# ramanathanlab/distllm

Measured on NVIDIA H100. Metric: embedded chunks/sec @512-tok, higher is better.
Workload: dtype bf16

## Files before the change

distllm_b200/_native.py:

```python

from __future__ import annotations

import ctypes as C
from pathlib import Path

import torch

LIB_PATH = Path(__file__).resolve().parent / 'libb2e.so'
LIB_PATHS = {'f16': LIB_PATH, 'bf16': LIB_PATH.with_name('libb2e_bf16.so')}
STORAGE_TORCH_DTYPE = {'f16': torch.float16, 'bf16': torch.bfloat16}
_STORAGE_BY_ARCH = {'bert': 'bf16', 'esm': 'bf16', 'modernbert': 'bf16', 'mistral': 'f16', 'qwen3': 'f16'}


def storage_for_arch(arch: str) -> str:
    import os

    forced = os.environ.get('B2E_STORAGE')
    if forced:
        if forced not in LIB_PATHS:
            raise NativeError(f'B2E_STORAGE={forced!r}: expected one of {sorted(LIB_PATHS)}')
        return forced
    return _STORAGE_BY_ARCH[arch]


# ... 17 lines not shown
    'b2e_num_weights',
    'b2e_check_model',
    'b2e_encoder_create',
    'b2e_encoder_create_nf4',
    'b2e_encoder_destroy',
    'b2e_workspace_bytes',
    'b2e_encode',
    'b2e_encode_pooled',
    'b2e_embed_host',
    'b2e_pool_mean',
    'b2e_pool_last_token',
    'b2e_l2_normalize',
    'b2e_adjacent_cosine_dist',
    'b2e_gemm_h16',
    'b2e_gemm_nf4',
    'b2e_attention_d64',
    'b2e_attention_d32',
    'b2e_attention_d64_window',
    'b2e_attention_causal_d128',
    'b2e_qk_norm_rope',
    'b2e_topk_ip',
    'b2e_topk_ip_tc',
    'b2e_max_row_norm',
    'b2e_pack_ubinary',
    'b2e_search_ubinary',
    'b2e_layernorm',
)
DEBUG_EXPORTS = (
    'b2e_debug_set_att3_clock',
    'b2e_debug_set_clock_buffer',
    'b2e_debug_set_layers',
    'b2e_debug_set_att3_variant',
    'b2e_debug_set_packing',
    'b2e_debug_topk_tc_fell_back',
)


class NativeError(RuntimeError):
    """Raised when libb2e.so is missing or a native call fails."""


class ModelDesc(C.Structure):

    _fields_ = [
        ('arch', C.c_int32),
        ('num_layers', C.c_int32),
        ('hidden', C.c_int32),
        ('heads', C.c_int32),
        ('kv_heads', C.c_int32),
        ('head_dim', C.c_int32),
        ('intermediate', C.c_int32),
        ('vocab', C.c_int32),
        ('max_pos', C.c_int32),
        ('type_vocab', C.c_int32),
        ('eps', C.c_float),
        ('rope_theta', C.c_float),
        ('sliding_window', C.c_int32),
        ('reserved', C.c_int32),
        ('rope_theta_local', C.c_float),
        ('global_every', C.c_int32),
    ]


_libs: dict[str, C.CDLL] = {}


# ... 385 lines not shown
```

distllm_b200/csrc/b2e_api.cu:

```cuda
#include "../../include/b2e.h"
#include "../../include/b2e_debug.h"

#include <cuda.h>
#include <cuda_runtime.h>

#include <cstdarg>
#include <cstdio>
#include <cstdlib>
#include <cstring>
#include <string>
#include <utility>
#include <vector>

#include "attention.cuh"
#include "binsearch.cuh"
#include "common.cuh"
#include "gemm.cuh"
#include "mistral_ops.cuh"
#include "pack.cuh"
#include "rowops.cuh"
#include "topk.cuh"
#include "topk_tc.cuh"

using namespace b2e;
// ... 127 lines not shown
  }
  static DeviceInfo cache[64];
  if (dev < 64 && cache[dev].ok) {
    *info = cache[dev];
    return B2E_OK;
  }
  int rc = device_info(dev, info);
  if (rc == B2E_OK && dev < 64) cache[dev] = *info;
  return rc;
}

template <typename Kern>
int ensure_smem_attr(Kern kern, int bytes) {
  static std::vector<std::pair<const void*, int>> done;
  int dev = 0;
  CUDA_TRY(cudaGetDevice(&dev));
  const void* key = reinterpret_cast<const void*>(kern);
  for (const auto& d : done)
    if (d.first == key && d.second == dev) return B2E_OK;
  CUDA_TRY(cudaFuncSetAttribute(kern, cudaFuncAttributeMaxDynamicSharedMemorySize, bytes));
  done.emplace_back(key, dev);
  return B2E_OK;
}

int check_gemm_shape(int M, int N, int K) {
  if (M <= 0 || N <= 0 || K <= 0) return fail(B2E_ERR_INVALID, "gemm: empty shape %dx%dx%d", M, N, K);
  if (N % 128 != 0) return fail(B2E_ERR_INVALID, "gemm: N=%d must be a multiple of 128", N);
  if (K % 64 != 0) return fail(B2E_ERR_INVALID, "gemm: K=%d must be a multiple of 64", K);
  return B2E_OK;
}

bool g_gemm_profiling = false;

struct GemmW {
  CUtensorMap tm;
  const float* absmax = nullptr;
};

int make_gemm_w(GemmW* w, const void* base, const float* absmax, uint64_t rows, uint64_t cols) {
  w->absmax = absmax;
  return absmax ? make_tmap_codes(&w->tm, base, rows, cols / 2) : make_tmap_h16(&w->tm, base, rows, cols, GEMM_BN);
}

template <int EPI>
int launch_gemm_epi(const CUtensorMap& ta, const GemmW& wb, void* out, const float* bias,
                    const h16* resid, int M, int N, int K, cudaStream_t st, const int* m_dev) {
  auto kern = gemm_h16_wgmma_kernel<EPI>;
  int smem = GEMM_SMEM_BYTES;
  if (wb.absmax) {
    kern = gemm_h16_wgmma_kernel<EPI, false, true>;
    smem = GemmPlan<true>::SMEM_BYTES;
  } else if constexpr (EPI == EPI_BIAS) {
    if (g_gemm_profiling) kern = gemm_h16_wgmma_kernel<EPI, true>;
  }
  int rc = ensure_smem_attr(kern, smem);
  if (rc) return rc;
  DeviceInfo dev;
  if ((rc = current_device_info(&dev))) return rc;
  const long long tiles = (long long)(N / GEMM_BN) * ((M + GEMM_BM - 1) / GEMM_BM);
  if (tiles > 0x7fffffffLL) return fail(B2E_ERR_INVALID, "gemm: %lld output tiles exceed one grid", tiles);
  CUtensorMap tm_out;
  if ((rc = make_tmap_h16(&tm_out, out, M, epi_is_glu(EPI) ? N / 2 : N, GEMM_BM))) return rc;
  const unsigned grid = (unsigned)(tiles < dev.sms ? tiles : dev.sms);
  kern<<<grid, GEMM_THREADS, smem, st>>>(ta, wb.tm, tm_out, static_cast<h16*>(out), bias, resid, M, N, K, m_dev,
                                         wb.absmax);
  CUDA_TRY(cudaGetLastError());
  return B2E_OK;
}

int launch_gemm(const CUtensorMap& ta, const GemmW& tb, void* out, const float* bias,
                const void* resid, int M, int N, int K, int epi, cudaStream_t st, const int* m_dev = nullptr) {
  const h16* r = static_cast<const h16*>(resid);
  switch (epi) {
    case B2E_EPI_BIAS: return launch_gemm_epi<EPI_BIAS>(ta, tb, out, bias, r, M, N, K, st, m_dev);
    case B2E_EPI_BIAS_GELU: return launch_gemm_epi<EPI_BIAS_GELU>(ta, tb, out, bias, r, M, N, K, st, m_dev);
    case B2E_EPI_BIAS_RESID: return launch_gemm_epi<EPI_BIAS_RESID>(ta, tb, out, bias, r, M, N, K, st, m_dev);
    case B2E_EPI_SWIGLU: return launch_gemm_epi<EPI_SWIGLU>(ta, tb, out, bias, r, M, N, K, st, m_dev);
    case B2E_EPI_GEGLU: return launch_gemm_epi<EPI_GEGLU>(ta, tb, out, bias, r, M, N, K, st, m_dev);
  }
  return fail(B2E_ERR_INVALID, "unknown epilogue %d", epi);
}

struct AttnScratch {
  float* bias = nullptr;
  int* kv_chunks = nullptr;
  int* plain_chunks = nullptr;
  size_t cap_bias = 0, cap_b = 0;
  uint64_t gen = 0;
  int device = -1;
  int ensure(int B, int S_pad) {
    int dev = 0;
    CUDA_TRY(cudaGetDevice(&dev));
// ... 599 lines not shown
      return rc;
    if ((rc = launch_gemm(tm_ffn, e->tm_w2[l], e->tmp, nullptr, nullptr, M, H, I, B2E_EPI_BIAS, st, lay.t_real)))
      return rc;
  }
  CUDA_TRY(cudaGetLastError());
  return B2E_OK;
}

}

extern "C" {

int b2e_version(void) { return B2E_ABI_VERSION; }
int b2e_storage_dtype(void) { return kStorageDtype; }

int b2e_debug_set_att3_clock(void* device_buffer) {
  long long* p = static_cast<long long*>(device_buffer);
  CUDA_TRY(cudaMemcpyToSymbol(g_att_clock, &p, sizeof(p)));
  return B2E_OK;
}

int b2e_debug_set_att3_variant(int variant) {
  g_att3_variant = variant;
  return B2E_OK;
}

int b2e_debug_set_clock_buffer(void* device_buffer) {
  long long* p = static_cast<long long*>(device_buffer);
  g_gemm_profiling = p != nullptr;
  CUDA_TRY(cudaMemcpyToSymbol(g_gemm_clock, &p, sizeof(p)));
  return B2E_OK;
}

int b2e_debug_set_packing(int on) {
  g_packing = on ? 1 : 0;
  return B2E_OK;
}

int b2e_debug_set_layers(B2EEncoder* e, int n) {
  if (!e) return fail(B2E_ERR_INVALID, "null encoder handle");
  if (n == 0) n = e->full_layers;
  if (n < 1 || n > e->full_layers)
    return fail(B2E_ERR_INVALID, "layer count %d outside [1, %d]", n, e->full_layers);
  if (n != e->desc.num_layers) e->drop_graphs();
  e->desc.num_layers = n;
  return B2E_OK;
}
const char* b2e_last_error(void) { return g_err.c_str(); }

int b2e_num_weights(const B2EModelDesc* desc) {
  if (!desc) return -1;
  if (desc->arch == B2E_ARCH_BERT) return 5 + 12 * desc->num_layers;
  if (desc->arch == B2E_ARCH_ESM2) return 3 + 12 * desc->num_layers;
  if (is_decoder(desc->arch)) return 2 + decoder_layer_slots(desc->arch) * desc->num_layers;
  if (desc->arch == B2E_ARCH_MODERNBERT) return 5 + 8 * desc->num_layers;
  return -1;
}

int b2e_check_model(const B2EModelDesc* desc) {
  if (!desc) return fail(B2E_ERR_INVALID, "null model description");
  if (desc->num_layers <= 0 || desc->hidden <= 0 || desc->heads <= 0 || desc->intermediate <= 0)
    return fail(B2E_ERR_INVALID, "model description has a non-positive size");
  int rc;
  if (is_decoder(desc->arch)) {
    const char* fam = desc->arch == B2E_ARCH_QWEN3 ? "Qwen3" : "Mistral";
    if (desc->head_dim != 128 || desc->kv_heads <= 0 || desc->heads % desc->kv_heads != 0)
// ... 34 lines not shown
                "{1,2,3,4,5,8,10,16}, 384 and 640 (MiniLM / BGE-small / E5-small: 384 = 12 x 32); of the ESM-2 family "
                "that is esm2_t30_150M (H=640), esm2_t33_650M (H=1280) and esm2_t36_3B (H=2560)",
                desc->heads, desc->head_dim, desc->hidden);
  if ((rc = check_h(desc->hidden))) return rc;
  if ((rc = check_gemm_shape(128, 3 * desc->hidden, desc->hidden))) return rc;
  if ((rc = check_gemm_shape(128, desc->intermediate, desc->hidden))) return rc;
  return check_gemm_shape(128, desc->hidden, desc->intermediate);
}

namespace {
int create_mistral(const B2EModelDesc* desc, const void* const* weights, int n_weights, const float* const* absmax,
                   int device, B2EEncoder** out) {
  const int L = desc->num_layers, H = desc->hidden, I = desc->intermediate;
  const int QC = (desc->heads + 2 * desc->kv_heads) * 128, CC = desc->heads * 128;
  int rc;
  if ((rc = b2e_check_model(desc))) return rc;
  if (n_weights != b2e_num_weights(desc))
    return fail(B2E_ERR_INVALID, "expected %d weight pointers, got %d", b2e_num_weights(desc), n_weights);
  for (int i = 0; i < n_weights; ++i)
    if (!weights[i]) return fail(B2E_ERR_INVALID, "weight pointer %d is null", i);
  DeviceInfo info;
  if ((rc = device_info(device, &info))) return rc;
  DeviceGuard guard;
  CUDA_TRY(cudaSetDevice(device));
  B2EEncoder* e = new B2EEncoder();
  e->desc = *desc;
  e->full_layers = desc->num_layers;
  e->w.assign(weights, weights + n_weights);
  e->device = device;
  e->sms = info.sms;
  e->tm_wqkv.resize(L); e->tm_wo.resize(L); e->tm_w1.resize(L); e->tm_w2.resize(L);
  for (int l = 0; l < L; ++l) {
    const float* const* s = absmax ? absmax + 4 * l : nullptr;
    if ((rc = make_gemm_w(&e->tm_wqkv[l], e->Mi(l, 1), s ? s[0] : nullptr, QC, H)) ||
        (rc = make_gemm_w(&e->tm_wo[l], e->Mi(l, 2), s ? s[1] : nullptr, H, CC)) ||
        (rc = make_gemm_w(&e->tm_w1[l], e->Mi(l, 4), s ? s[2] : nullptr, 2 * I, H)) ||
        (rc = make_gemm_w(&e->tm_w2[l], e->Mi(l, 5), s ? s[3] : nullptr, H, I))) {
      delete e;
      return rc;
    }
  }
  const size_t n = (size_t)desc->max_pos * 64;
  if (cudaMalloc(&e->rope_cos, n * sizeof(float)) != cudaSuccess ||
      cudaMalloc(&e->rope_sin, n * sizeof(float)) != cudaSuccess) {
    b2e_encoder_destroy(e);
    return fail(B2E_ERR_CUDA, "cudaMalloc of the rotary tables failed");
  }
  rope_table_theta_kernel<<<(unsigned)((n + 255) / 256), 256>>>(e->rope_cos, e->rope_sin, desc->max_pos,
                                                                64, desc->rope_theta);
  if (cudaDeviceSynchronize() != cudaSuccess) {
    b2e_encoder_destroy(e);
    return fail(B2E_ERR_CUDA, "rotary table kernel failed: %s", cudaGetErrorString(cudaGetLastError()));
  }
  *out = e;
  return B2E_OK;
}
}

namespace {
int create_encoder(const B2EModelDesc* desc, const void* const* weights, int n_weights, const float* const* absmax,
                   int device, B2EEncoder** out) {
  if (!desc || !weights || !out) return fail(B2E_ERR_INVALID, "null argument");
  *out = nullptr;
  if (is_decoder(desc->arch)) return create_mistral(desc, weights, n_weights, absmax, device, out);
  int rc;
  if ((rc = b2e_check_model(desc))) return rc;
  if (n_weights != b2e_num_weights(desc))
    return fail(B2E_ERR_INVALID, "expected %d weight pointers, got %d", b2e_num_weights(desc),
                n_weights);
  for (int i = 0; i < n_weights; ++i)
    if (!weights[i]) return fail(B2E_ERR_INVALID, "weight pointer %d is null", i);
  DeviceInfo info;
  if ((rc = device_info(device, &info))) return rc;
  DeviceGuard guard;
  CUDA_TRY(cudaSetDevice(device));

  B2EEncoder* e = new B2EEncoder();
  e->desc = *desc;
  e->full_layers = desc->num_layers;
  e->w.assign(weights, weights + n_weights);
  e->device = device;
  e->sms = info.sms;
  const int L = desc->num_layers, H = desc->hidden, I = desc->intermediate;
  e->tm_wqkv.resize(L); e->tm_wo.resize(L); e->tm_w1.resize(L); e->tm_w2.resize(L);
  const bool esm = desc->arch == B2E_ARCH_ESM2;
  const bool mbert = desc->arch == B2E_ARCH_MODERNBERT;
  const int n1 = mbert ? 2 * I : I;
  for (int l = 0; l < L; ++l) {
    const void* wqkv = mbert ? e->Mb(l, 2) : esm ? e->E(l, 2) : e->L(l, 0);
    const void* wo = mbert ? e->Mb(l, 3) : esm ? e->E(l, 4) : e->L(l, 2);
    const void* w1 = mbert ? e->Mb(l, 6) : esm ? e->E(l, 8) : e->L(l, 6);
    const void* w2 = mbert ? e->Mb(l, 7) : esm ? e->E(l, 10) : e->L(l, 8);
    const float* const* s = absmax ? absmax + 4 * l : nullptr;
    if ((rc = make_gemm_w(&e->tm_wqkv[l], wqkv, s ? s[0] : nullptr, 3 * H, H)) ||
        (rc = make_gemm_w(&e->tm_wo[l], wo, s ? s[1] : nullptr, H, H)) ||
        (rc = make_gemm_w(&e->tm_w1[l], w1, s ? s[2] : nullptr, n1, H)) ||
        (rc = make_gemm_w(&e->tm_w2[l], w2, s ? s[3] : nullptr, H, I))) {
      delete e;
      return rc;
    }
  }
  if (mbert) {
    const size_t n = (size_t)desc->max_pos * 32;
    if (cudaMalloc(&e->rope_cos, n * sizeof(float)) != cudaSuccess ||
        cudaMalloc(&e->rope_sin, n * sizeof(float)) != cudaSuccess ||
        cudaMalloc(&e->rope_cos2, n * sizeof(float)) != cudaSuccess ||
        cudaMalloc(&e->rope_sin2, n * sizeof(float)) != cudaSuccess) {
      b2e_encoder_destroy(e);
      return fail(B2E_ERR_CUDA, "cudaMalloc of the rotary tables failed");
    }
    rope_table_theta_kernel<<<(unsigned)((n + 255) / 256), 256>>>(e->rope_cos, e->rope_sin, desc->max_pos, 32,
                                                                  desc->rope_theta);
    rope_table_theta_kernel<<<(unsigned)((n + 255) / 256), 256>>>(e->rope_cos2, e->rope_sin2, desc->max_pos, 32,
                                                                  desc->rope_theta_local);
    if (cudaDeviceSynchronize() != cudaSuccess) {
      b2e_encoder_destroy(e);
      return fail(B2E_ERR_CUDA, "rotary table kernel failed: %s", cudaGetErrorString(cudaGetLastError()));
    }
  }
  if (esm) {
    const size_t n = (size_t)desc->max_pos * 32;
    if (cudaMalloc(&e->rope_cos, n * sizeof(float)) != cudaSuccess ||
        cudaMalloc(&e->rope_sin, n * sizeof(float)) != cudaSuccess) {
      b2e_encoder_destroy(e);
      return fail(B2E_ERR_CUDA, "cudaMalloc of the rotary tables failed");
    }
    if (desc->head_dim == 32)
      rope_table_theta_kernel<<<(unsigned)((n / 2 + 255) / 256), 256>>>(e->rope_cos, e->rope_sin, desc->max_pos, 16,
                                                                        10000.0f);
    else
// ... 371 lines not shown
  switch (dtype) {
    case B2E_DTYPE_F32:
      adjacent_cosine_kernel<float><<<blocks, 256, 0, st>>>((const float*)emb, doc_id, out,
                                                            (int)n_rows, H);
      break;
    case B2E_DTYPE_BF16:
      adjacent_cosine_kernel<bf16><<<blocks, 256, 0, st>>>((const bf16*)emb, doc_id, out,
                                                           (int)n_rows, H);
      break;
    case B2E_DTYPE_F16:
      adjacent_cosine_kernel<__half><<<blocks, 256, 0, st>>>((const __half*)emb, doc_id, out,
                                                             (int)n_rows, H);
      break;
    default:
      return fail(B2E_ERR_INVALID, "adjacent_cosine_dist: dtype %d", dtype);
  }
  CUDA_TRY(cudaGetLastError());
  return B2E_OK;
}

int b2e_gemm_h16(const void* A, const void* W, const float* bias, const void* resid, void* out,
                  int M, int N, int K, int epi, void* stream) {
  if (!A || !W || !out) return fail(B2E_ERR_INVALID, "null tensor pointer");
  if (epi == B2E_EPI_BIAS_RESID && !resid) return fail(B2E_ERR_INVALID, "resid epilogue needs resid");
  int rc;
  if ((rc = check_gemm_shape(M, N, K))) return rc;
  if ((epi == B2E_EPI_SWIGLU || epi == B2E_EPI_GEGLU) && N % 256 != 0)
    return fail(B2E_ERR_INVALID, "gemm: the gated epilogues need N %% 256 == 0 (got %d)", N);
  DeviceInfo info;
  if ((rc = current_device_info(&info))) return rc;
  CUtensorMap ta;
  GemmW tb;
  if ((rc = make_tmap_h16(&ta, A, M, K, 128))) return rc;
  if ((rc = make_gemm_w(&tb, W, nullptr, N, K))) return rc;
  return launch_gemm(ta, tb, out, bias, resid, M, N, K, epi, (cudaStream_t)stream);
}

int b2e_gemm_nf4(const void* A, const void* codes, const float* absmax, const float* bias, const void* resid,
                 void* out, int M, int N, int K, int epi, void* stream) {
  if (!A || !codes || !absmax || !out) return fail(B2E_ERR_INVALID, "null tensor pointer");
  if (reinterpret_cast<uintptr_t>(absmax) % 16 != 0) return fail(B2E_ERR_INVALID, "absmax not 16-byte aligned");
  if (epi == B2E_EPI_BIAS_RESID && !resid) return fail(B2E_ERR_INVALID, "resid epilogue needs resid");
  int rc;
  if ((rc = check_gemm_shape(M, N, K))) return rc;
  if ((epi == B2E_EPI_SWIGLU || epi == B2E_EPI_GEGLU) && N % 256 != 0)
    return fail(B2E_ERR_INVALID, "gemm: the gated epilogues need N %% 256 == 0 (got %d)", N);
  DeviceInfo info;
  if ((rc = current_device_info(&info))) return rc;
  CUtensorMap ta;
  GemmW tb;
  if ((rc = make_tmap_h16(&ta, A, M, K, 128))) return rc;
  if ((rc = make_gemm_w(&tb, codes, absmax, N, K))) return rc;
  return launch_gemm(ta, tb, out, bias, resid, M, N, K, epi, (cudaStream_t)stream);
}

int b2e_attention_d64(const void* qkv, const int64_t* mask, void* ctx, int B, int S, int heads,
                      float* dbg, void* stream) {
  if (!qkv || !mask || !ctx) return fail(B2E_ERR_INVALID, "null tensor pointer");
  if (B <= 0 || S <= 0 || heads <= 0) return fail(B2E_ERR_INVALID, "empty attention problem");
  if (dbg) return fail(B2E_ERR_UNSUPPORTED, "the score dump of the first attention kernel is gone: pass NULL");
  int rc;
  DeviceInfo info;
  if ((rc = current_device_info(&info))) return rc;
  cudaStream_t st = (cudaStream_t)stream;
  CUtensorMap tkv;
  if ((rc = make_tmap_h16(&tkv, qkv, (uint64_t)B * S, (uint64_t)3 * heads * 64, AT_KC))) return rc;
  if ((rc = attention_prepare(g_attn_scratch, mask, B, S, st))) return rc;
  return launch_attention(tkv, g_attn_scratch, ctx, B, S, heads, st);
}

int b2e_attention_d32(const void* qkv, const int64_t* mask, void* ctx, int B, int S, int heads, void* stream) {
  if (!qkv || !mask || !ctx) return fail(B2E_ERR_INVALID, "null tensor pointer");
  if (B <= 0 || S <= 0 || heads <= 0) return fail(B2E_ERR_INVALID, "empty attention problem");
  int rc;
  DeviceInfo info;
  if ((rc = current_device_info(&info))) return rc;
  cudaStream_t st = (cudaStream_t)stream;
  CUtensorMap tkv;
  if ((rc = make_tmap_h16(&tkv, qkv, (uint64_t)B * S, (uint64_t)3 * heads * 32, AT_KC, 32))) return rc;
  if ((rc = attention_prepare(g_attn_scratch, mask, B, S, st))) return rc;
  return launch_attention_bidir(tkv, g_attn_scratch, ctx, B, S, heads, 32, st);
}

int b2e_attention_d64_window(const void* qkv, const int64_t* mask, void* ctx, int B, int S, int heads,
                             int window, void* stream) {
// ... 385 lines not shown
```

distllm_b200/csrc/common.cuh:

```cuda
#pragma once

#include <cuda.h>
#include <cuda_bf16.h>
#include <cuda_fp16.h>
#include <cuda_runtime.h>
#include <stdint.h>

namespace b2e {

using bf16 = __nv_bfloat16;
#ifdef B2E_STORAGE_BF16
using h16 = __nv_bfloat16;
#else
using h16 = __half;
#endif

__device__ __forceinline__ uint32_t smem_u32(const void* p) {
  return static_cast<uint32_t>(__cvta_generic_to_shared(p));
}

__device__ __forceinline__ uint32_t lane_id() { return threadIdx.x & 31u; }

__device__ __forceinline__ bool elect_one() {
  uint32_t pred = 0;
// ... 186 lines not shown
        "+f"(d[24]), "+f"(d[25]), "+f"(d[26]), "+f"(d[27]), "+f"(d[28]), "+f"(d[29]), "+f"(d[30]), "+f"(d[31])
      : "r"(a[0]), "r"(a[1]), "r"(a[2]), "r"(a[3]), "l"(b));
}

__device__ __forceinline__ void wgmma_64x32_rs_tb(float (&d)[16], const uint32_t (&a)[4], uint64_t b) {
  asm volatile(
      "{\n.reg .pred p;\nsetp.eq.u32 p, 1, 1;\n"
      "wgmma.mma_async.sync.aligned.m64n32k16.f32." B2E_WGMMA_AB " "
      "{%0,%1,%2,%3,%4,%5,%6,%7,%8,%9,%10,%11,%12,%13,%14,%15}, {%16,%17,%18,%19}, %20, p, 1, 1, 1;\n}\n"
      : "+f"(d[0]), "+f"(d[1]), "+f"(d[2]), "+f"(d[3]), "+f"(d[4]), "+f"(d[5]), "+f"(d[6]), "+f"(d[7]),
        "+f"(d[8]), "+f"(d[9]), "+f"(d[10]), "+f"(d[11]), "+f"(d[12]), "+f"(d[13]), "+f"(d[14]), "+f"(d[15])
      : "r"(a[0]), "r"(a[1]), "r"(a[2]), "r"(a[3]), "l"(b));
}

__device__ __forceinline__ void wgmma_64x128_ss(float (&d)[64], uint64_t a, uint64_t b, int accumulate) {
  asm volatile(
      "{\n.reg .pred p;\nsetp.ne.b32 p, %66, 0;\n"
      "wgmma.mma_async.sync.aligned.m64n128k16.f32." B2E_WGMMA_AB " "
      "{%0,%1,%2,%3,%4,%5,%6,%7,%8,%9,%10,%11,%12,%13,%14,%15,"
      "%16,%17,%18,%19,%20,%21,%22,%23,%24,%25,%26,%27,%28,%29,%30,%31,"
      "%32,%33,%34,%35,%36,%37,%38,%39,%40,%41,%42,%43,%44,%45,%46,%47,"
      "%48,%49,%50,%51,%52,%53,%54,%55,%56,%57,%58,%59,%60,%61,%62,%63}, %64, %65, p, 1, 1, 0, 0;\n}\n"
      : "+f"(d[0]), "+f"(d[1]), "+f"(d[2]), "+f"(d[3]), "+f"(d[4]), "+f"(d[5]), "+f"(d[6]), "+f"(d[7]),
        "+f"(d[8]), "+f"(d[9]), "+f"(d[10]), "+f"(d[11]), "+f"(d[12]), "+f"(d[13]), "+f"(d[14]), "+f"(d[15]),
        "+f"(d[16]), "+f"(d[17]), "+f"(d[18]), "+f"(d[19]), "+f"(d[20]), "+f"(d[21]), "+f"(d[22]), "+f"(d[23]),
        "+f"(d[24]), "+f"(d[25]), "+f"(d[26]), "+f"(d[27]), "+f"(d[28]), "+f"(d[29]), "+f"(d[30]), "+f"(d[31]),
        "+f"(d[32]), "+f"(d[33]), "+f"(d[34]), "+f"(d[35]), "+f"(d[36]), "+f"(d[37]), "+f"(d[38]), "+f"(d[39]),
        "+f"(d[40]), "+f"(d[41]), "+f"(d[42]), "+f"(d[43]), "+f"(d[44]), "+f"(d[45]), "+f"(d[46]), "+f"(d[47]),
        "+f"(d[48]), "+f"(d[49]), "+f"(d[50]), "+f"(d[51]), "+f"(d[52]), "+f"(d[53]), "+f"(d[54]), "+f"(d[55]),
        "+f"(d[56]), "+f"(d[57]), "+f"(d[58]), "+f"(d[59]), "+f"(d[60]), "+f"(d[61]), "+f"(d[62]), "+f"(d[63])
      : "l"(a), "l"(b), "r"(accumulate));
}

__device__ __forceinline__ void wgmma_64x16_tf32(float (&d)[8], uint64_t a, uint64_t b, int accumulate) {
  asm volatile(
      "{\n.reg .pred p;\nsetp.ne.b32 p, %10, 0;\n"
      "wgmma.mma_async.sync.aligned.m64n16k8.f32.tf32.tf32 {%0,%1,%2,%3,%4,%5,%6,%7}, %8, %9, p, 1, 1;\n}\n"
      : "+f"(d[0]), "+f"(d[1]), "+f"(d[2]), "+f"(d[3]), "+f"(d[4]), "+f"(d[5]), "+f"(d[6]), "+f"(d[7])
      : "l"(a), "l"(b), "r"(accumulate));
}


__device__ __forceinline__ uint32_t pack_h16x2(float lo, float hi) {
  uint32_t r;
#ifdef B2E_STORAGE_BF16
  asm("cvt.rn.bf16x2.f32 %0, %1, %2;" : "=r"(r) : "f"(hi), "f"(lo));
#else
  asm("cvt.rn.satfinite.f16x2.f32 %0, %1, %2;" : "=r"(r) : "f"(hi), "f"(lo));
#endif
  return r;
}
__device__ __forceinline__ float2 unpack_h16x2(uint32_t u) {
#ifdef B2E_STORAGE_BF16
  __nv_bfloat162 v = *reinterpret_cast<__nv_bfloat162*>(&u);
  return __bfloat1622float2(v);
#else
  __half2 v = *reinterpret_cast<__half2*>(&u);
  return __half22float2(v);
#endif
}
__device__ __forceinline__ float2 unpack_bf16x2(uint32_t u) {
  __nv_bfloat162 v = *reinterpret_cast<__nv_bfloat162*>(&u);
  return __bfloat1622float2(v);
}
__device__ __forceinline__ h16 to_h16(float x) {
#ifdef B2E_STORAGE_BF16
// ... 32 lines not shown
```

distllm_b200/csrc/gemm.cuh:

```cuda
#pragma once

#include "common.cuh"

namespace b2e {

enum GemmEpi : int { EPI_BIAS = 0, EPI_BIAS_GELU = 1, EPI_BIAS_RESID = 2, EPI_SWIGLU = 3, EPI_GEGLU = 4 };
__host__ __device__ constexpr bool epi_is_glu(int epi) { return epi == EPI_SWIGLU || epi == EPI_GEGLU; }

constexpr int GEMM_BM = 128;
constexpr int GEMM_BN = 128;
constexpr int GEMM_BK = 64;
constexpr int GEMM_STAGES = 5;
constexpr int GEMM_THREADS = 384;
constexpr int GEMM_PRODUCER_REGS = 40, GEMM_CONSUMER_REGS = 232;
constexpr int GEMM_A_BYTES = GEMM_BM * GEMM_BK * 2;
constexpr int GEMM_STAGE_BYTES = GEMM_A_BYTES + GEMM_BN * GEMM_BK * 2;
constexpr int GEMM_OUT_BOX = GEMM_BM * 64 * 2;
constexpr int GEMM_OUT_OFFSET = GEMM_STAGES * GEMM_STAGE_BYTES;
constexpr int GEMM_BAR_OFFSET = GEMM_OUT_OFFSET + 2 * 2 * GEMM_OUT_BOX;
constexpr int GEMM_SMEM_BYTES = GEMM_BAR_OFFSET + 16 * GEMM_STAGES + 1024;
static_assert(GEMM_SMEM_BYTES <= 232448, "shared memory of one SM");
constexpr int GEMM_BAR_TURN = 1, GEMM_BAR_STAGE = 3, GEMM_BAR_NF4 = 5;

constexpr int GEMM_NF4_RAW = 4;
constexpr int GEMM_NF4_CODE_BYTES = GEMM_BN * GEMM_BK / 2;
constexpr int GEMM_NF4_RAW_BYTES = GEMM_NF4_CODE_BYTES + GEMM_BN * 4;

template <bool NF4>
struct GemmPlan {
  static constexpr int STAGES = NF4 ? 4 : GEMM_STAGES;
  static constexpr int OUT_OFFSET = STAGES * GEMM_STAGE_BYTES;
  static constexpr int RAW_OFFSET = OUT_OFFSET + 2 * 2 * GEMM_OUT_BOX;
  static constexpr int BAR_OFFSET = RAW_OFFSET + (NF4 ? GEMM_NF4_RAW * GEMM_NF4_RAW_BYTES : 0);
  static constexpr int TABLE_OFFSET = BAR_OFFSET + 16 * STAGES + (NF4 ? 8 * GEMM_NF4_RAW : 0);
  static constexpr int SMEM_BYTES = TABLE_OFFSET + (NF4 ? 16 * 4 : 0) + 1024;
  static constexpr int PRODUCER_REGS = NF4 ? 56 : GEMM_PRODUCER_REGS;
  static constexpr int CONSUMER_REGS = NF4 ? 224 : GEMM_CONSUMER_REGS;
  static_assert(128 * PRODUCER_REGS + 256 * CONSUMER_REGS <= GEMM_THREADS * 168, "registers the CTA holds");
  static_assert(SMEM_BYTES <= 232448, "shared memory of one SM");
};
static_assert(GemmPlan<false>::SMEM_BYTES == GEMM_SMEM_BYTES && GemmPlan<false>::BAR_OFFSET == GEMM_BAR_OFFSET,
              "the 16-bit plan");

__constant__ uint32_t kNf4CodeBits[16] = {
    0xbf800000u, 0xbf3239b1u, 0xbf066b30u, 0xbeca32a0u, 0xbe91a24du, 0xbe3d353fu, 0xbdba7871u, 0x00000000u,
    0x3da2faffu, 0x3e24cae3u, 0x3e7c04ddu, 0x3ead033au, 0x3ee1a4b8u, 0x3f1007abu, 0x3f3913b3u, 0x3f800000u,
};

__device__ __forceinline__ float gelu_erf_fast(float x) {
  const float xc = fminf(fmaxf(x, -5.65685f), 5.65685f);
  const float v = xc * xc;
  float q = fmaf(v, -1.35688221e-05f, -1.95764464e-04f);
  q = fmaf(v, q, 3.65498251e-02f);
  q = fmaf(v, q, 7.97818838e-01f);
  float t;
  asm("tanh.approx.f32 %0, %1;" : "=f"(t) : "f"(xc * q));
  const float h = 0.5f * x;
  return fmaf(h, t, h);
}

__device__ __forceinline__ float gelu_erf(float x) {
  const float ax = fabsf(x);
  float t;
  asm("rcp.approx.ftz.f32 %0, %1;" : "=f"(t) : "f"(fmaf(0.3275911f * 0.70710678f, ax, 1.0f)));
  float p = fmaf(t, 1.061405429f, -1.453152027f);
  p = fmaf(t, p, 1.421413741f);
  p = fmaf(t, p, -0.284496736f);
  p = fmaf(t, p, 0.254829592f);
  p *= t;
  const float e = fast_exp2(ax * ax * (-0.5f * 1.4426950408889634f));
  return fmaxf(x, 0.0f) - 0.5f * ax * p * e;
}

__device__ __forceinline__ float silu(float x) {
  float r;
  asm("rcp.approx.ftz.f32 %0, %1;" : "=f"(r) : "f"(1.0f + fast_exp2(-1.4426950408889634f * x)));
  return x * r;
}


__device__ long long* g_gemm_clock = nullptr;

struct GemmTiles {
  int first, stride, count, n_tiles;
};
__device__ __forceinline__ GemmTiles gemm_tiles(int M, int N) {
  const int n_tiles = N / GEMM_BN;
  const int tiles = n_tiles * ((M + GEMM_BM - 1) / GEMM_BM);
  const int first = static_cast<int>(blockIdx.x), stride = static_cast<int>(gridDim.x);
  return {first, stride, first < tiles ? (tiles - 1 - first) / stride + 1 : 0, n_tiles};
}

__device__ __forceinline__ float ld_shared_const_f32(uint32_t addr) {
  float v;
  asm("ld.shared.f32 %0, [%1];" : "=f"(v) : "r"(addr));
  return v;
}
__device__ __forceinline__ float ld_shared_f32(uint32_t addr) {
  float v;
  asm volatile("ld.shared.f32 %0, [%1];" : "=f"(v) : "r"(addr) : "memory");
  return v;
}
__device__ __forceinline__ uint4 ld_shared_v4(uint32_t addr) {
  uint4 v;
  asm volatile("ld.shared.v4.u32 {%0, %1, %2, %3}, [%4];" : "=r"(v.x), "=r"(v.y), "=r"(v.z), "=r"(v.w) : "r"(addr)
               : "memory");
  return v;
}
__device__ __forceinline__ void st_shared_v4(uint32_t addr, uint32_t a, uint32_t b, uint32_t c, uint32_t d) {
  asm volatile("st.shared.v4.b32 [%0], {%1, %2, %3, %4};" ::"r"(addr), "r"(a), "r"(b), "r"(c), "r"(d) : "memory");
}

__device__ __forceinline__ void gemm_nf4_producer(const CUtensorMap* tm_a, const CUtensorMap* tm_codes,
                                                  const float* __restrict__ absmax, const GemmTiles& tl, int N,
                                                  int kblocks, uint32_t sb, uint32_t full_bar, uint32_t empty_bar) {
  using P = GemmPlan<true>;
  const int p = static_cast<int>(threadIdx.x) - 256;
  const uint32_t raw0 = sb + P::RAW_OFFSET;
  const uint32_t raw_bar = empty_bar + 8u * P::STAGES;
  const uint32_t table = sb + P::TABLE_OFFSET;
// ... 27 lines not shown
        mbar_expect_tx(fb, GEMM_A_BYTES);
        tma_load_2d(dst, tm_a, fb, kb * GEMM_BK, m0);
      }
      mbar_wait(raw_bar + 8u * slot, raw_phase);
      const uint32_t src = raw0 + slot * GEMM_NF4_RAW_BYTES;
      const uint4 c0 = ld_shared_v4(src + 32 * p), c1 = ld_shared_v4(src + 32 * p + 16);
      const float s = ld_shared_f32(src + GEMM_NF4_CODE_BYTES + 4 * p);
      const uint32_t words[8] = {c0.x, c0.y, c0.z, c0.w, c1.x, c1.y, c1.z, c1.w};
      const uint32_t row = dst + GEMM_A_BYTES + 128 * p;
#pragma unroll
      for (int c = 0; c < 8; ++c) {
        uint32_t v[4];
#pragma unroll
        for (int b = 0; b < 4; ++b) {
          const uint32_t byte = (words[c] >> (8 * b)) & 0xffu;
          const float lo = __fmul_rn(ld_shared_const_f32(table + ((byte >> 4) << 2)), s);
          const float hi = __fmul_rn(ld_shared_const_f32(table + ((byte & 15u) << 2)), s);
          v[b] = pack_h16x2(lo, hi);
        }
        st_shared_v4(row + ((c ^ (p & 7)) << 4), v[0], v[1], v[2], v[3]);
      }
      fence_proxy_async_smem();
      named_bar_sync(GEMM_BAR_NF4, 128);
      if (p == 0) {
        mbar_arrive(fb);
        if (ld < total) load_raw();
      }
      if (++stage == P::STAGES) { stage = 0; phase ^= 1u; }
      if (++slot == GEMM_NF4_RAW) { slot = 0; raw_phase ^= 1u; }
    }
  }
}

template <int EPI, bool TL = false, bool NF4 = false>
__global__ void __launch_bounds__(GEMM_THREADS, 1)
gemm_h16_wgmma_kernel(const __grid_constant__ CUtensorMap tm_a,
                      const __grid_constant__ CUtensorMap tm_b,
                      const __grid_constant__ CUtensorMap tm_out,
                      h16* __restrict__ out, const float* __restrict__ bias, const h16* __restrict__ resid,
                      int M, int N, int K, const int* __restrict__ m_dev, const float* __restrict__ absmax) {
  using P = GemmPlan<NF4>;
  if (m_dev != nullptr) M = __ldg(m_dev);
  const GemmTiles tl = gemm_tiles(M, N);
  extern __shared__ uint8_t smem_raw[];
  const uint32_t sb = (smem_u32(smem_raw) + 1023u) & ~1023u;
  const uint32_t full_bar = sb + P::BAR_OFFSET;
  const uint32_t empty_bar = full_bar + 8u * P::STAGES;
  const int warp = threadIdx.x >> 5;
  const int kblocks = K / GEMM_BK;

  if (threadIdx.x == 0) {
    for (int s = 0; s < P::STAGES; ++s) {
      mbar_init(full_bar + 8u * s, NF4 ? 2 : 1);
      mbar_init(empty_bar + 8u * s, 1);
    }
    if constexpr (NF4)
      for (int s = 0; s < GEMM_NF4_RAW; ++s) mbar_init(empty_bar + 8u * (P::STAGES + s), 1);
    mbar_fence_init();
  }
  if constexpr (NF4)
    if (threadIdx.x < 16) st_shared_u32(sb + P::TABLE_OFFSET + 4 * threadIdx.x, kNf4CodeBits[threadIdx.x]);
  __syncthreads();

  long long* clk = (TL && blockIdx.x == 0) ? g_gemm_clock : nullptr;
  if (warp >= 8) {
    asm volatile("setmaxnreg.dec.sync.aligned.u32 %0;" ::"n"(P::PRODUCER_REGS));
    if constexpr (NF4) {
      gemm_nf4_producer(&tm_a, &tm_b, absmax, tl, N, kblocks, sb, full_bar, empty_bar);
    } else if (warp == 8 && elect_one()) {
      tma_prefetch_desc(&tm_a);
      tma_prefetch_desc(&tm_b);
      int stage = 0, n = 0;
      uint32_t phase = 0;
      for (int i = 0; i < tl.count; ++i) {
        const int tile = tl.first + i * tl.stride;
        const int m0 = (tile / tl.n_tiles) * GEMM_BM, n0 = (tile % tl.n_tiles) * GEMM_BN;
        for (int kb = 0; kb < kblocks; ++kb, ++n) {
          mbar_wait(empty_bar + 8u * stage, phase ^ 1u);
          const uint32_t dst = sb + stage * GEMM_STAGE_BYTES;
          const uint32_t fb = full_bar + 8u * stage;
          mbar_expect_tx(fb, GEMM_STAGE_BYTES);
          tma_load_2d(dst, &tm_a, fb, kb * GEMM_BK, m0);
          tma_load_2d(dst + GEMM_A_BYTES, &tm_b, fb, kb * GEMM_BK, n0);
          if (TL && clk != nullptr && n < 256) clk[n] = clock64();
          if (++stage == GEMM_STAGES) { stage = 0; phase ^= 1u; }
        }
      }
    }
    return;
  }

  asm volatile("setmaxnreg.inc.sync.aligned.u32 %0;" ::"n"(P::CONSUMER_REGS));
  const int wg = warp >> 2;
  const int t = threadIdx.x & 127;
  const int quad = t & 3;
  const int r_lo = 16 * (t >> 5) + ((t & 31) >> 2);
  const uint32_t stg = sb + P::OUT_OFFSET + wg * (2 * GEMM_OUT_BOX);
  int retired = 0;
  for (int i = wg; i < tl.count; i += 2) {
    const int tile = tl.first + i * tl.stride;
    const int m0 = (tile / tl.n_tiles) * GEMM_BM, n_blk = tile % tl.n_tiles;
    float acc[2][64];
#pragma unroll
    for (int x = 0; x < 64; ++x) acc[0][x] = acc[1][x] = 0.0f;
    if (i > 0) named_bar_sync(GEMM_BAR_TURN + wg, 256);
    const int it = i * kblocks;
    int stage = it % P::STAGES;
    uint32_t phase = (it / P::STAGES) & 1u;
    int prev = -1;
    for (int kb = 0; kb < kblocks; ++kb) {
      mbar_wait(full_bar + 8u * stage, phase);
      const uint32_t a_addr = sb + stage * GEMM_STAGE_BYTES;
      const uint64_t a0 = make_smem_desc_sw128(a_addr), a1 = make_smem_desc_sw128(a_addr + 64 * 128);
      const uint64_t b_desc = make_smem_desc_sw128(a_addr + GEMM_A_BYTES);
      reg_fence(acc[0]);
      reg_fence(acc[1]);
      wgmma_fence();
#pragma unroll
      for (int k = 0; k < GEMM_BK / 16; ++k) {
        wgmma_64x128_ss(acc[0], a0 + 2u * k, b_desc + 2u * k, (kb | k) != 0);
        wgmma_64x128_ss(acc[1], a1 + 2u * k, b_desc + 2u * k, (kb | k) != 0);
      }
      wgmma_commit();
      reg_fence(acc[0]);
      reg_fence(acc[1]);
      wgmma_wait<1>();
      reg_fence(acc[0]);
      reg_fence(acc[1]);
      if (prev >= 0 && t == 0) mbar_arrive(empty_bar + 8u * prev);
      if (TL && clk != nullptr && wg == 0 && t == 0 && retired < 256) clk[256 + retired] = clock64();
      ++retired;
      prev = stage;
      if (++stage == P::STAGES) { stage = 0; phase ^= 1u; }
    }
    if (i + 1 < tl.count) named_bar_arrive(GEMM_BAR_TURN + (wg ^ 1), 256);
    wgmma_wait<0>();
    reg_fence(acc[0]);
    reg_fence(acc[1]);
    if (t == 0) mbar_arrive(empty_bar + 8u * prev);

    const bool staged = m0 + GEMM_BM <= M;
    if (staged) {
      if (t == 0) tma_store_wait_read<0>();
      named_bar_sync(GEMM_BAR_STAGE + wg, 128);
    }
    if constexpr (epi_is_glu(EPI)) {
      const int n_out = N / 2;
#pragma unroll
      for (int j = 0; j < 8; ++j)
#pragma unroll
        for (int h = 0; h < 2; ++h)
#pragma unroll
          for (int half = 0; half < 2; ++half) {
            const int r = 64 * h + r_lo + 8 * half;
            const float g0 = acc[h][4 * j + 2 * half], g1 = acc[h][4 * j + 2 * half + 1];
            const float u0 = acc[h][4 * (j + 8) + 2 * half], u1 = acc[h][4 * (j + 8) + 2 * half + 1];
            float v0, v1;
            if (EPI == EPI_GEGLU) {
              v0 = gelu_erf_fast(g0) * u0;
              v1 = gelu_erf_fast(g1) * u1;
            } else {
              v0 = silu(g0) * u0;
              v1 = silu(g1) * u1;
            }
            if (staged)
              st_shared_u32(stg + r * 128 + ((j ^ (r & 7)) << 4) + 4 * quad, pack_h16x2(v0, v1));
            else if (m0 + r < M)
              *reinterpret_cast<uint32_t*>(out + static_cast<size_t>(m0 + r) * n_out + n_blk * (GEMM_BN / 2) +
                                           8 * j + 2 * quad) = pack_h16x2(v0, v1);
          }
    } else {
      const int col0 = n_blk * GEMM_BN + 2 * quad;
#pragma unroll
      for (int j = 0; j < 16; ++j) {
        const float2 b = bias != nullptr ? __ldg(reinterpret_cast<const float2*>(bias + col0 + 8 * j))
                                         : make_float2(0.0f, 0.0f);
#pragma unroll
        for (int h = 0; h < 2; ++h)
#pragma unroll
          for (int half = 0; half < 2; ++half) {
            const int r = 64 * h + r_lo + 8 * half;
            if (!staged && m0 + r >= M) continue;
            float v0 = acc[h][4 * j + 2 * half], v1 = acc[h][4 * j + 2 * half + 1];
            if (bias != nullptr) {
              v0 += b.x;
              v1 += b.y;
            }
            if (EPI == EPI_BIAS_GELU) {
              v0 = gelu_erf_fast(v0);
              v1 = gelu_erf_fast(v1);
            }
            const size_t off = static_cast<size_t>(m0 + r) * N + col0 + 8 * j;
            if (EPI == EPI_BIAS_RESID) {
              const float2 rv = unpack_h16x2(*reinterpret_cast<const uint32_t*>(resid + off));
              v0 += rv.x;
              v1 += rv.y;
            }
            if (staged)
              st_shared_u32(stg + (j >> 3) * GEMM_OUT_BOX + r * 128 + (((j & 7) ^ (r & 7)) << 4) + 4 * quad,
                            pack_h16x2(v0, v1));
            else
              *reinterpret_cast<uint32_t*>(out + off) = pack_h16x2(v0, v1);
          }
      }
    }
    if (staged) {
      fence_proxy_async_smem();
      named_bar_sync(GEMM_BAR_STAGE + wg, 128);
      if (t == 0) {
        if constexpr (epi_is_glu(EPI)) {
          tma_store_2d(&tm_out, stg, n_blk * (GEMM_BN / 2), m0);
        } else {
          tma_store_2d(&tm_out, stg, n_blk * GEMM_BN, m0);
          tma_store_2d(&tm_out, stg + GEMM_OUT_BOX, n_blk * GEMM_BN + 64, m0);
        }
        tma_store_commit();
      }
    }
  }
  if (t == 0) tma_store_wait_all();
}

}
```

include/b2e_debug.h:

```cpp
#ifndef B2E_DEBUG_H_
#define B2E_DEBUG_H_

#ifdef __cplusplus
extern "C" {
#endif

struct B2EEncoder;
int b2e_debug_set_layers(struct B2EEncoder* enc, int n_layers);

int b2e_debug_set_att3_clock(void* device_buffer);
int b2e_debug_set_att3_variant(int variant);
int b2e_debug_set_clock_buffer(void* device_buffer);
int b2e_debug_set_packing(int on);
int b2e_debug_topk_tc_fell_back(int* out);

#ifdef __cplusplus
}
#endif
#endif
```

Before: 4180.

## Add 192-wide GEMM tiles for non-gated 16-bit weight GEMMs

Adds a BN=192 variant of the warp-specialized wgmma GEMM, using m64n192k16 instructions, a 3-stage pipeline, larger consumer register budgets and three TMA output boxes. It is selected by default for non-NF4, non-gated epilogues when N is divisible by 192. Wider tiles raise the arithmetic intensity per loaded A tile and reduce tile count. The cost is fewer pipeline stages, heavier register pressure, and possible wave-quantization changes on the SM grid.

```diff
diff --git a/distllm_b200/_native.py b/distllm_b200/_native.py
--- a/distllm_b200/_native.py
+++ b/distllm_b200/_native.py
@@ -73,6 +73,8 @@
     'b2e_debug_set_layers',
     'b2e_debug_set_att3_variant',
     'b2e_debug_set_packing',
+    'b2e_debug_set_gemm_bn',
+    'b2e_debug_gemm_bn',
     'b2e_debug_topk_tc_fell_back',
 )
 
diff --git a/distllm_b200/csrc/b2e_api.cu b/distllm_b200/csrc/b2e_api.cu
--- a/distllm_b200/csrc/b2e_api.cu
+++ b/distllm_b200/csrc/b2e_api.cu
@@ -183,14 +183,33 @@
 
 bool g_gemm_profiling = false;
 
+int g_gemm_bn = -1;
+inline int gemm_bn_override() {
+  if (g_gemm_bn < 0) {
+    const char* e = getenv("B2E_GEMM_BN");
+    const int v = e ? atoi(e) : 0;
+    g_gemm_bn = (v == 128 || v == 192) ? v : 0;
+  }
+  return g_gemm_bn;
+}
+
+int gemm_bn(int N, int epi, bool nf4) {
+  const bool wide_ok = !nf4 && epi != B2E_EPI_SWIGLU && epi != B2E_EPI_GEGLU && N % 192 == 0;
+  if (!wide_ok) return 128;
+  const int forced = gemm_bn_override();
+  return forced ? forced : 192;
+}
+
 struct GemmW {
   CUtensorMap tm;
   const float* absmax = nullptr;
+  int bn = GEMM_BN;
 };
 
-int make_gemm_w(GemmW* w, const void* base, const float* absmax, uint64_t rows, uint64_t cols) {
+int make_gemm_w(GemmW* w, const void* base, const float* absmax, uint64_t rows, uint64_t cols, int epi) {
   w->absmax = absmax;
-  return absmax ? make_tmap_codes(&w->tm, base, rows, cols / 2) : make_tmap_h16(&w->tm, base, rows, cols, GEMM_BN);
+  w->bn = gemm_bn((int)rows, epi, absmax != nullptr);
+  return absmax ? make_tmap_codes(&w->tm, base, rows, cols / 2) : make_tmap_h16(&w->tm, base, rows, cols, w->bn);
 }
 
 template <int EPI>
@@ -198,9 +217,19 @@
                     const h16* resid, int M, int N, int K, cudaStream_t st, const int* m_dev) {
   auto kern = gemm_h16_wgmma_kernel<EPI>;
   int smem = GEMM_SMEM_BYTES;
+  if (N % wb.bn != 0) return fail(B2E_ERR_INVALID, "gemm: N=%d is not a multiple of its W map's tile width %d", N, wb.bn);
   if (wb.absmax) {
     kern = gemm_h16_wgmma_kernel<EPI, false, true>;
     smem = GemmPlan<true>::SMEM_BYTES;
+  } else if (wb.bn == 192) {
+    if constexpr (epi_is_glu(EPI)) {
+      return fail(B2E_ERR_INVALID, "gemm: the gated epilogues run 128-wide tiles only");
+    } else {
+      kern = gemm_h16_wgmma_kernel<EPI, false, false, 192>;
+      smem = GemmPlan<false, 192>::SMEM_BYTES;
+      if constexpr (EPI == EPI_BIAS)
+        if (g_gemm_profiling) kern = gemm_h16_wgmma_kernel<EPI, true, false, 192>;
+    }
   } else if constexpr (EPI == EPI_BIAS) {
     if (g_gemm_profiling) kern = gemm_h16_wgmma_kernel<EPI, true>;
   }
@@ -208,7 +237,7 @@
   if (rc) return rc;
   DeviceInfo dev;
   if ((rc = current_device_info(&dev))) return rc;
-  const long long tiles = (long long)(N / GEMM_BN) * ((M + GEMM_BM - 1) / GEMM_BM);
+  const long long tiles = (long long)(N / wb.bn) * ((M + GEMM_BM - 1) / GEMM_BM);
   if (tiles > 0x7fffffffLL) return fail(B2E_ERR_INVALID, "gemm: %lld output tiles exceed one grid", tiles);
   CUtensorMap tm_out;
   if ((rc = make_tmap_h16(&tm_out, out, M, epi_is_glu(EPI) ? N / 2 : N, GEMM_BM))) return rc;
@@ -874,6 +903,18 @@
   return B2E_OK;
 }
 
+int b2e_debug_set_gemm_bn(int bn) {
+  if (bn != 0 && bn != 128 && bn != 192) return fail(B2E_ERR_INVALID, "gemm tile width %d: 0, 128 or 192", bn);
+  g_gemm_bn = bn;
+  return B2E_OK;
+}
+
+int b2e_debug_gemm_bn(int n, int epi, int nf4, int* out) {
+  if (!out) return fail(B2E_ERR_INVALID, "null argument");
+  *out = gemm_bn(n, epi, nf4 != 0);
+  return B2E_OK;
+}
+
 int b2e_debug_set_packing(int on) {
   g_packing = on ? 1 : 0;
   return B2E_OK;
@@ -974,10 +1015,10 @@
   e->tm_wqkv.resize(L); e->tm_wo.resize(L); e->tm_w1.resize(L); e->tm_w2.resize(L);
   for (int l = 0; l < L; ++l) {
     const float* const* s = absmax ? absmax + 4 * l : nullptr;
-    if ((rc = make_gemm_w(&e->tm_wqkv[l], e->Mi(l, 1), s ? s[0] : nullptr, QC, H)) ||
-        (rc = make_gemm_w(&e->tm_wo[l], e->Mi(l, 2), s ? s[1] : nullptr, H, CC)) ||
-        (rc = make_gemm_w(&e->tm_w1[l], e->Mi(l, 4), s ? s[2] : nullptr, 2 * I, H)) ||
-        (rc = make_gemm_w(&e->tm_w2[l], e->Mi(l, 5), s ? s[3] : nullptr, H, I))) {
+    if ((rc = make_gemm_w(&e->tm_wqkv[l], e->Mi(l, 1), s ? s[0] : nullptr, QC, H, B2E_EPI_BIAS)) ||
+        (rc = make_gemm_w(&e->tm_wo[l], e->Mi(l, 2), s ? s[1] : nullptr, H, CC, B2E_EPI_BIAS)) ||
+        (rc = make_gemm_w(&e->tm_w1[l], e->Mi(l, 4), s ? s[2] : nullptr, 2 * I, H, B2E_EPI_SWIGLU)) ||
+        (rc = make_gemm_w(&e->tm_w2[l], e->Mi(l, 5), s ? s[3] : nullptr, H, I, B2E_EPI_BIAS))) {
       delete e;
       return rc;
     }
@@ -1034,10 +1075,10 @@
     const void* w1 = mbert ? e->Mb(l, 6) : esm ? e->E(l, 8) : e->L(l, 6);
     const void* w2 = mbert ? e->Mb(l, 7) : esm ? e->E(l, 10) : e->L(l, 8);
     const float* const* s = absmax ? absmax + 4 * l : nullptr;
-    if ((rc = make_gemm_w(&e->tm_wqkv[l], wqkv, s ? s[0] : nullptr, 3 * H, H)) ||
-        (rc = make_gemm_w(&e->tm_wo[l], wo, s ? s[1] : nullptr, H, H)) ||
-        (rc = make_gemm_w(&e->tm_w1[l], w1, s ? s[2] : nullptr, n1, H)) ||
-        (rc = make_gemm_w(&e->tm_w2[l], w2, s ? s[3] : nullptr, H, I))) {
+    if ((rc = make_gemm_w(&e->tm_wqkv[l], wqkv, s ? s[0] : nullptr, 3 * H, H, B2E_EPI_BIAS)) ||
+        (rc = make_gemm_w(&e->tm_wo[l], wo, s ? s[1] : nullptr, H, H, B2E_EPI_BIAS)) ||
+        (rc = make_gemm_w(&e->tm_w1[l], w1, s ? s[2] : nullptr, n1, H, mbert ? B2E_EPI_GEGLU : B2E_EPI_BIAS_GELU)) ||
+        (rc = make_gemm_w(&e->tm_w2[l], w2, s ? s[3] : nullptr, H, I, B2E_EPI_BIAS))) {
       delete e;
       return rc;
     }
@@ -1475,7 +1516,7 @@
   CUtensorMap ta;
   GemmW tb;
   if ((rc = make_tmap_h16(&ta, A, M, K, 128))) return rc;
-  if ((rc = make_gemm_w(&tb, W, nullptr, N, K))) return rc;
+  if ((rc = make_gemm_w(&tb, W, nullptr, N, K, epi))) return rc;
   return launch_gemm(ta, tb, out, bias, resid, M, N, K, epi, (cudaStream_t)stream);
 }
 
@@ -1493,7 +1534,7 @@
   CUtensorMap ta;
   GemmW tb;
   if ((rc = make_tmap_h16(&ta, A, M, K, 128))) return rc;
-  if ((rc = make_gemm_w(&tb, codes, absmax, N, K))) return rc;
+  if ((rc = make_gemm_w(&tb, codes, absmax, N, K, epi))) return rc;
   return launch_gemm(ta, tb, out, bias, resid, M, N, K, epi, (cudaStream_t)stream);
 }
 
diff --git a/distllm_b200/csrc/common.cuh b/distllm_b200/csrc/common.cuh
--- a/distllm_b200/csrc/common.cuh
+++ b/distllm_b200/csrc/common.cuh
@@ -242,6 +242,31 @@
       : "l"(a), "l"(b), "r"(accumulate));
 }
 
+__device__ __forceinline__ void wgmma_64x192_ss(float (&d)[96], uint64_t a, uint64_t b, int accumulate) {
+  asm volatile(
+      "{\n.reg .pred p;\nsetp.ne.b32 p, %98, 0;\n"
+      "wgmma.mma_async.sync.aligned.m64n192k16.f32." B2E_WGMMA_AB " "
+      "{%0,%1,%2,%3,%4,%5,%6,%7,%8,%9,%10,%11,%12,%13,%14,%15,"
+      "%16,%17,%18,%19,%20,%21,%22,%23,%24,%25,%26,%27,%28,%29,%30,%31,"
+      "%32,%33,%34,%35,%36,%37,%38,%39,%40,%41,%42,%43,%44,%45,%46,%47,"
+      "%48,%49,%50,%51,%52,%53,%54,%55,%56,%57,%58,%59,%60,%61,%62,%63,"
+      "%64,%65,%66,%67,%68,%69,%70,%71,%72,%73,%74,%75,%76,%77,%78,%79,"
+      "%80,%81,%82,%83,%84,%85,%86,%87,%88,%89,%90,%91,%92,%93,%94,%95}, %96, %97, p, 1, 1, 0, 0;\n}\n"
+      : "+f"(d[0]), "+f"(d[1]), "+f"(d[2]), "+f"(d[3]), "+f"(d[4]), "+f"(d[5]), "+f"(d[6]), "+f"(d[7]),
+        "+f"(d[8]), "+f"(d[9]), "+f"(d[10]), "+f"(d[11]), "+f"(d[12]), "+f"(d[13]), "+f"(d[14]), "+f"(d[15]),
+        "+f"(d[16]), "+f"(d[17]), "+f"(d[18]), "+f"(d[19]), "+f"(d[20]), "+f"(d[21]), "+f"(d[22]), "+f"(d[23]),
+        "+f"(d[24]), "+f"(d[25]), "+f"(d[26]), "+f"(d[27]), "+f"(d[28]), "+f"(d[29]), "+f"(d[30]), "+f"(d[31]),
+        "+f"(d[32]), "+f"(d[33]), "+f"(d[34]), "+f"(d[35]), "+f"(d[36]), "+f"(d[37]), "+f"(d[38]), "+f"(d[39]),
+        "+f"(d[40]), "+f"(d[41]), "+f"(d[42]), "+f"(d[43]), "+f"(d[44]), "+f"(d[45]), "+f"(d[46]), "+f"(d[47]),
+        "+f"(d[48]), "+f"(d[49]), "+f"(d[50]), "+f"(d[51]), "+f"(d[52]), "+f"(d[53]), "+f"(d[54]), "+f"(d[55]),
+        "+f"(d[56]), "+f"(d[57]), "+f"(d[58]), "+f"(d[59]), "+f"(d[60]), "+f"(d[61]), "+f"(d[62]), "+f"(d[63]),
+        "+f"(d[64]), "+f"(d[65]), "+f"(d[66]), "+f"(d[67]), "+f"(d[68]), "+f"(d[69]), "+f"(d[70]), "+f"(d[71]),
+        "+f"(d[72]), "+f"(d[73]), "+f"(d[74]), "+f"(d[75]), "+f"(d[76]), "+f"(d[77]), "+f"(d[78]), "+f"(d[79]),
+        "+f"(d[80]), "+f"(d[81]), "+f"(d[82]), "+f"(d[83]), "+f"(d[84]), "+f"(d[85]), "+f"(d[86]), "+f"(d[87]),
+        "+f"(d[88]), "+f"(d[89]), "+f"(d[90]), "+f"(d[91]), "+f"(d[92]), "+f"(d[93]), "+f"(d[94]), "+f"(d[95])
+      : "l"(a), "l"(b), "r"(accumulate));
+}
+
 __device__ __forceinline__ void wgmma_64x16_tf32(float (&d)[8], uint64_t a, uint64_t b, int accumulate) {
   asm volatile(
       "{\n.reg .pred p;\nsetp.ne.b32 p, %10, 0;\n"
diff --git a/distllm_b200/csrc/gemm.cuh b/distllm_b200/csrc/gemm.cuh
--- a/distllm_b200/csrc/gemm.cuh
+++ b/distllm_b200/csrc/gemm.cuh
@@ -26,21 +26,25 @@
 constexpr int GEMM_NF4_CODE_BYTES = GEMM_BN * GEMM_BK / 2;
 constexpr int GEMM_NF4_RAW_BYTES = GEMM_NF4_CODE_BYTES + GEMM_BN * 4;
 
-template <bool NF4>
+template <bool NF4, int BN = GEMM_BN>
 struct GemmPlan {
-  static constexpr int STAGES = NF4 ? 4 : GEMM_STAGES;
-  static constexpr int OUT_OFFSET = STAGES * GEMM_STAGE_BYTES;
-  static constexpr int RAW_OFFSET = OUT_OFFSET + 2 * 2 * GEMM_OUT_BOX;
+  static_assert(BN == 128 || BN == 192, "tile widths");
+  static_assert(!NF4 || BN == 128, "the NF4 producer writes one W row per thread of its warpgroup");
+  static constexpr int STAGE_BYTES = GEMM_A_BYTES + BN * GEMM_BK * 2;
+  static constexpr int OUT_BOXES = BN / 64;
+  static constexpr int STAGES = NF4 ? 4 : BN == 192 ? 3 : GEMM_STAGES;
+  static constexpr int OUT_OFFSET = STAGES * STAGE_BYTES;
+  static constexpr int RAW_OFFSET = OUT_OFFSET + 2 * OUT_BOXES * GEMM_OUT_BOX;
   static constexpr int BAR_OFFSET = RAW_OFFSET + (NF4 ? GEMM_NF4_RAW * GEMM_NF4_RAW_BYTES : 0);
   static constexpr int TABLE_OFFSET = BAR_OFFSET + 16 * STAGES + (NF4 ? 8 * GEMM_NF4_RAW : 0);
   static constexpr int SMEM_BYTES = TABLE_OFFSET + (NF4 ? 16 * 4 : 0) + 1024;
-  static constexpr int PRODUCER_REGS = NF4 ? 56 : GEMM_PRODUCER_REGS;
-  static constexpr int CONSUMER_REGS = NF4 ? 224 : GEMM_CONSUMER_REGS;
+  static constexpr int PRODUCER_REGS = NF4 ? 56 : BN == 192 ? 24 : GEMM_PRODUCER_REGS;
+  static constexpr int CONSUMER_REGS = NF4 ? 224 : BN == 192 ? 240 : GEMM_CONSUMER_REGS;
   static_assert(128 * PRODUCER_REGS + 256 * CONSUMER_REGS <= GEMM_THREADS * 168, "registers the CTA holds");
   static_assert(SMEM_BYTES <= 232448, "shared memory of one SM");
 };
-static_assert(GemmPlan<false>::SMEM_BYTES == GEMM_SMEM_BYTES && GemmPlan<false>::BAR_OFFSET == GEMM_BAR_OFFSET,
-              "the 16-bit plan");
+static_assert(GemmPlan<false>::SMEM_BYTES == GEMM_SMEM_BYTES && GemmPlan<false>::BAR_OFFSET == GEMM_BAR_OFFSET &&
+              GemmPlan<false>::STAGE_BYTES == GEMM_STAGE_BYTES, "the 16-bit plan");
 
 __constant__ uint32_t kNf4CodeBits[16] = {
     0xbf800000u, 0xbf3239b1u, 0xbf066b30u, 0xbeca32a0u, 0xbe91a24du, 0xbe3d353fu, 0xbdba7871u, 0x00000000u,
@@ -84,8 +88,9 @@
 struct GemmTiles {
   int first, stride, count, n_tiles;
 };
+template <int BN>
 __device__ __forceinline__ GemmTiles gemm_tiles(int M, int N) {
-  const int n_tiles = N / GEMM_BN;
+  const int n_tiles = N / BN;
   const int tiles = n_tiles * ((M + GEMM_BM - 1) / GEMM_BM);
   const int first = static_cast<int>(blockIdx.x), stride = static_cast<int>(gridDim.x);
   return {first, stride, first < tiles ? (tiles - 1 - first) / stride + 1 : 0, n_tiles};
@@ -179,16 +184,17 @@
   }
 }
 
-template <int EPI, bool TL = false, bool NF4 = false>
+template <int EPI, bool TL = false, bool NF4 = false, int BN = GEMM_BN>
 __global__ void __launch_bounds__(GEMM_THREADS, 1)
 gemm_h16_wgmma_kernel(const __grid_constant__ CUtensorMap tm_a,
                       const __grid_constant__ CUtensorMap tm_b,
                       const __grid_constant__ CUtensorMap tm_out,
                       h16* __restrict__ out, const float* __restrict__ bias, const h16* __restrict__ resid,
                       int M, int N, int K, const int* __restrict__ m_dev, const float* __restrict__ absmax) {
-  using P = GemmPlan<NF4>;
+  using P = GemmPlan<NF4, BN>;
+  static_assert(!epi_is_glu(EPI) || BN == 128, "the gated epilogues pair gate and up within a 128-row W tile");
   if (m_dev != nullptr) M = __ldg(m_dev);
-  const GemmTiles tl = gemm_tiles(M, N);
+  const GemmTiles tl = gemm_tiles<BN>(M, N);
   extern __shared__ uint8_t smem_raw[];
   const uint32_t sb = (smem_u32(smem_raw) + 1023u) & ~1023u;
   const uint32_t full_bar = sb + P::BAR_OFFSET;
@@ -221,16 +227,16 @@
       uint32_t phase = 0;
       for (int i = 0; i < tl.count; ++i) {
         const int tile = tl.first + i * tl.stride;
-        const int m0 = (tile / tl.n_tiles) * GEMM_BM, n0 = (tile % tl.n_tiles) * GEMM_BN;
+        const int m0 = (tile / tl.n_tiles) * GEMM_BM, n0 = (tile % tl.n_tiles) * BN;
         for (int kb = 0; kb < kblocks; ++kb, ++n) {
           mbar_wait(empty_bar + 8u * stage, phase ^ 1u);
-          const uint32_t dst = sb + stage * GEMM_STAGE_BYTES;
+          const uint32_t dst = sb + stage * P::STAGE_BYTES;
           const uint32_t fb = full_bar + 8u * stage;
-          mbar_expect_tx(fb, GEMM_STAGE_BYTES);
+          mbar_expect_tx(fb, P::STAGE_BYTES);
           tma_load_2d(dst, &tm_a, fb, kb * GEMM_BK, m0);
           tma_load_2d(dst + GEMM_A_BYTES, &tm_b, fb, kb * GEMM_BK, n0);
           if (TL && clk != nullptr && n < 256) clk[n] = clock64();
-          if (++stage == GEMM_STAGES) { stage = 0; phase ^= 1u; }
+          if (++stage == P::STAGES) { stage = 0; phase ^= 1u; }
         }
       }
     }
@@ -242,14 +248,14 @@
   const int t = threadIdx.x & 127;
   const int quad = t & 3;
   const int r_lo = 16 * (t >> 5) + ((t & 31) >> 2);
-  const uint32_t stg = sb + P::OUT_OFFSET + wg * (2 * GEMM_OUT_BOX);
+  const uint32_t stg = sb + P::OUT_OFFSET + wg * (P::OUT_BOXES * GEMM_OUT_BOX);
   int retired = 0;
   for (int i = wg; i < tl.count; i += 2) {
     const int tile = tl.first + i * tl.stride;
     const int m0 = (tile / tl.n_tiles) * GEMM_BM, n_blk = tile % tl.n_tiles;
-    float acc[2][64];
-#pragma unroll
-    for (int x = 0; x < 64; ++x) acc[0][x] = acc[1][x] = 0.0f;
+    float acc[2][BN / 2];
+#pragma unroll
+    for (int x = 0; x < BN / 2; ++x) acc[0][x] = acc[1][x] = 0.0f;
     if (i > 0) named_bar_sync(GEMM_BAR_TURN + wg, 256);
     const int it = i * kblocks;
     int stage = it % P::STAGES;
@@ -257,7 +263,7 @@
     int prev = -1;
     for (int kb = 0; kb < kblocks; ++kb) {
       mbar_wait(full_bar + 8u * stage, phase);
-      const uint32_t a_addr = sb + stage * GEMM_STAGE_BYTES;
+      const uint32_t a_addr = sb + stage * P::STAGE_BYTES;
       const uint64_t a0 = make_smem_desc_sw128(a_addr), a1 = make_smem_desc_sw128(a_addr + 64 * 128);
       const uint64_t b_desc = make_smem_desc_sw128(a_addr + GEMM_A_BYTES);
       reg_fence(acc[0]);
@@ -265,8 +271,13 @@
       wgmma_fence();
 #pragma unroll
       for (int k = 0; k < GEMM_BK / 16; ++k) {
-        wgmma_64x128_ss(acc[0], a0 + 2u * k, b_desc + 2u * k, (kb | k) != 0);
-        wgmma_64x128_ss(acc[1], a1 + 2u * k, b_desc + 2u * k, (kb | k) != 0);
+        if constexpr (BN == 192) {
+          wgmma_64x192_ss(acc[0], a0 + 2u * k, b_desc + 2u * k, (kb | k) != 0);
+          wgmma_64x192_ss(acc[1], a1 + 2u * k, b_desc + 2u * k, (kb | k) != 0);
+        } else {
+          wgmma_64x128_ss(acc[0], a0 + 2u * k, b_desc + 2u * k, (kb | k) != 0);
+          wgmma_64x128_ss(acc[1], a1 + 2u * k, b_desc + 2u * k, (kb | k) != 0);
+        }
       }
       wgmma_commit();
       reg_fence(acc[0]);
@@ -317,9 +328,9 @@
                                            8 * j + 2 * quad) = pack_h16x2(v0, v1);
           }
     } else {
-      const int col0 = n_blk * GEMM_BN + 2 * quad;
-#pragma unroll
-      for (int j = 0; j < 16; ++j) {
+      const int col0 = n_blk * BN + 2 * quad;
+#pragma unroll
+      for (int j = 0; j < BN / 8; ++j) {
         const float2 b = bias != nullptr ? __ldg(reinterpret_cast<const float2*>(bias + col0 + 8 * j))
                                          : make_float2(0.0f, 0.0f);
 #pragma unroll
@@ -358,8 +369,8 @@
         if constexpr (epi_is_glu(EPI)) {
           tma_store_2d(&tm_out, stg, n_blk * (GEMM_BN / 2), m0);
         } else {
-          tma_store_2d(&tm_out, stg, n_blk * GEMM_BN, m0);
-          tma_store_2d(&tm_out, stg + GEMM_OUT_BOX, n_blk * GEMM_BN + 64, m0);
+#pragma unroll
+          for (int b = 0; b < P::OUT_BOXES; ++b) tma_store_2d(&tm_out, stg + b * GEMM_OUT_BOX, n_blk * BN + 64 * b, m0);
         }
         tma_store_commit();
       }
diff --git a/include/b2e_debug.h b/include/b2e_debug.h
--- a/include/b2e_debug.h
+++ b/include/b2e_debug.h
@@ -11,6 +11,8 @@
 int b2e_debug_set_att3_clock(void* device_buffer);
 int b2e_debug_set_att3_variant(int variant);
 int b2e_debug_set_clock_buffer(void* device_buffer);
+int b2e_debug_set_gemm_bn(int bn);
+int b2e_debug_gemm_bn(int n, int epi, int nf4, int* out);
 int b2e_debug_set_packing(int on);
 int b2e_debug_topk_tc_fell_back(int* out);
 
```

Result: faster. 4443, median of 6 (+6.3%).
